# tum-pbs/differentiable-piso

Hardware: AMD Instinct MI355X
Metric: PISO steps/s (fwd+adjoint) at 2048^2 staggered grid (higher is better)
Workload: dtype f64

## Files before the change

### differentiable-piso_amd/csrc/cg.hip

```cpp
#include <atomic>
#include "cg_kernels.h"
#include "cg_driver.h"
#include "cg_tiny.h"
#include "options.h"
#include <cstdio>
#include <vector>

namespace piso {

struct CgProfile {
  int enabled = 0, stride = 8;
  double ms[4] = {0, 0, 0, 0};
  long long count[4] = {0, 0, 0, 0};
};
static CgProfile g_prof;

struct HostPoll {
  CgState* pinned = nullptr;
  hipEvent_t ev[2] = {nullptr, nullptr};
  hipEvent_t seg_ev[2] = {nullptr, nullptr};
  int cus = 0;
};
static std::atomic<unsigned> g_persist_launches{0};
static int g_persist_fallbacks = 0;
static thread_local int tl_xcd_map[kPersistMaxGrid];
static thread_local int tl_xcd_map_n = 0;
static long long g_tiny_solves = 0;
enum { DI_PATH = 0, DI_SIZEOF_T, DI_SIZEOF_CT, DI_V, DI_RECON, DI_SYMMETRIC, DI_ROWS_PER_WAVE, DI_K1_GRID, DI_K1_TILES, DI_R, DI_NQ,
       DI_WAVES, DI_LAUNCH_GRID, DI_PADDED, DI_XCD_LOCAL, DI_FELL_BACK, DI_TINY_PER_X, DI_K2_GRID, DI_SEGMENTS, DI_COUNT };
static thread_local int tl_dispatch[DI_COUNT];
static thread_local int tl_dispatch_n = 0;
static bool g_xcd_local_failed = false;
static long long g_verify_runs = 0;
static int g_verify_failures = 0;
constexpr int kPollDevices = 16;
static thread_local HostPoll tl_poll_dev[kPollDevices];
static thread_local HostPoll* tl_poll_cur = &tl_poll_dev[0];
#define tl_poll (*tl_poll_cur)

static int ensure_poll() {
  int dev = 0;
// ... 185 lines not shown
    if (prof) PISO_TRY(ensure_events(ep));
    ep.used[0] = ep.used[1] = 0;
    prof_stride = g_prof.stride > 0 ? g_prof.stride : 8;
    cg_init<T><<<tile.gflat, kBlock, 0, stream>>>(a, rank_deficient);
    PISO_LAUNCH_CHECK();
    batch = poll_batch(n);
    plan = persist_plan(PersistQuery{a.nx, a.ny, V, a.per_y, a.nx_true != 0, sizeof(T), sizeof(CT), RECON, symmetric, false, tl_poll.cus,
                                     opt(OPT_CG_PERSIST), opt(OPT_CG_PERSIST_R), opt(OPT_CG_PERSIST_HALF), opt(OPT_CG_PERSIST_NQ),
                                     opt(OPT_CG_XCD_LOCAL), g_xcd_local_failed, allow_persist});
    PISO_TRY((persist_prepare<T, CT, RECON, false>(plan, tl_poll.cus, pc, persist_ws, stream)));
    if (plan.R && kPersistDiag && opt_on(OPT_CG_PERSIST_TIMING)) {
      PISO_HIP_CHECK(hipMalloc(reinterpret_cast<void**>(&timing.ticks), 12 * plan.launch_grid * sizeof(unsigned long long)));
      PISO_HIP_CHECK(hipMemsetAsync(timing.ticks, 0, 12 * plan.launch_grid * sizeof(unsigned long long), stream));
      pc.timing = timing.ticks;
    }
    record_dispatch(plan.R ? 3 : 2, sizeof(T), sizeof(CT), 0, V, RECON, symmetric, &tile, &plan, !allow_persist);
    seg_len = persist_segment_len(n, opt(OPT_CG_SEGMENT));
    hipEvent_t* seg_ev = tl_poll.seg_ev;
    if (plan.R && prof && !seg_ev[0]) { PISO_HIP_CHECK(hipEventCreate(&seg_ev[0])); PISO_HIP_CHECK(hipEventCreate(&seg_ev[1])); }
    return PISO_OK;
  }

  bool persistent() const { return plan.R != 0; }
  int segment(int k, int ke, CgLoop& st) {
    hipEvent_t* seg_ev = tl_poll.seg_ev;
    if (prof) PISO_HIP_CHECK(hipEventRecord(seg_ev[0], stream));
    PISO_TRY((persist_launch<T, CT, RECON, false>(plan, a, pc, g_persist_launches.fetch_add(1, std::memory_order_relaxed), k, ke, st.sv, st.pending, NoSlab{}, stream)));
    if (prof) PISO_HIP_CHECK(hipEventRecord(seg_ev[1], stream));
    const bool defer = !prof && ke - k <= 32 && unsynced + (ke - k) <= 256 && ke < st.total;
    unsynced = defer ? unsynced + (ke - k) : 0;
// ... 48 lines not shown
  int look(int k, CgLoop& st) { return (!fixed && (k + 1) % batch == 0 && k + 1 < st.total) ? poll(st, false) : PISO_OK; }

  int finish(CgLoop& st) {
    if (!fixed && !st.finished) PISO_TRY(poll(st, true));
    PISO_HIP_CHECK(hipStreamSynchronize(stream));
    if (opt(OPT_CG_XCD_MAP) == 1) {
      tl_xcd_map_n = 0;
      if (st.segments_run > 0 && !plan.xcd_local && plan.grid <= kPersistMaxGrid) {
        PISO_HIP_CHECK(hipMemcpy(tl_xcd_map, pc.xcd + kPersistXcdTable, (size_t)plan.grid * sizeof(int), hipMemcpyDeviceToHost));
        tl_xcd_map_n = plan.grid;
      }
    }
    if (st.segments_run > 0) {
      int herr = 0;
      PISO_HIP_CHECK(hipMemcpy(&herr, pc.err, sizeof(int), hipMemcpyDeviceToHost));
      if (herr) { ++g_persist_fallbacks; return kPersistRetry; }
    }
    if (st.segments_run > 0 && sizeof(T) == 8 && !fixed && opt(OPT_CG_VERIFY) != 0) {
      bool failed = false;
      PISO_TRY((verify_residual<T, CT>(a, pc, stream, &failed)));
      if (failed) { ++g_verify_failures; ++g_persist_fallbacks; return kPersistRetry; }
    }
    if (timing.ticks) PISO_TRY(print_persist_timing(timing.ticks, plan.grid, st.k_last));
    tl_dispatch[DI_SEGMENTS] = st.segments_run;
    return PISO_OK;
  }
};

template <typename T>
__global__ __launch_bounds__(kBlock) void cg_copy_rows(const T* __restrict__ src, T* __restrict__ dst, int nx, int ny, int ld_src, int ld_dst) {
// ... 161 lines not shown
                                 const double* divergence, double* x_out, int rank_deficient, int iterations,
                                 float* kernel_ms_out, void* workspace, size_t workspace_bytes, piso_stream_t stream) {
  const piso::OptScope knobs;
  if (iterations < 1) { set_error_msg("piso_cg_fixed_iterations: iterations < 1"); return PISO_ERR_INVALID_ARG; }
  return cg_solve<double>(nx, ny, periodic_x, periodic_y, laplace, divergence, x_out, 0.f, iterations, rank_deficient,
                          1 << 30, iterations, nullptr, kernel_ms_out, workspace, workspace_bytes, stream);
}

void piso_cg_profile_enable(int enable, int stride) {
  g_prof.enabled = enable;
  if (stride > 0) g_prof.stride = stride;
  for (int q = 0; q < 4; ++q) { g_prof.ms[q] = 0; g_prof.count[q] = 0; }
}

int piso_cg_persist_fallbacks(void) { return g_persist_fallbacks; }
int piso_cg_last_xcd_map(int* out, int capacity) {
  const int n = tl_xcd_map_n < capacity ? tl_xcd_map_n : capacity;
  for (int i = 0; i < n; ++i) out[i] = tl_xcd_map[i];
  return tl_xcd_map_n;
}
long long piso_cg_tiny_solves(void) { return g_tiny_solves; }
int piso_cg_last_dispatch(int* out, int capacity) {
  const int n = tl_dispatch_n < capacity ? tl_dispatch_n : capacity;
  for (int i = 0; i < n; ++i) out[i] = tl_dispatch[i];
  return tl_dispatch_n;
}
void piso_cg_verify_stats(long long* runs_out, int* failures_out) {
  if (runs_out) *runs_out = g_verify_runs;
  if (failures_out) *failures_out = g_verify_failures;
}
// ... 7 lines not shown
```

### differentiable-piso_amd/csrc/cg_dispatch.h

```cpp
#pragma once
#include <type_traits>

#include "cg_persist1.h"

namespace piso {

constexpr int kXcdCus = 32;
constexpr int kPersistRetry = -1000;

struct CgTiling { int rows_per_wave, k1_tiles, g1, g2, gflat; };
template <typename T>
inline CgTiling cg_tile(CgArgs<T>& a, int V, int rpw_knob, int maxblocks_knob) {
  const size_t n = (size_t)a.nx * a.ny;
  a.ntx = (a.nx + 64 * V - 1) / (64 * V);
  int rpw = (int)(((long long)a.ny * a.ntx) / (4 * 1024));
  rpw = rpw < 2 ? 2 : (rpw > 16 ? 16 : rpw);
  if (rpw_knob > 0) rpw = rpw_knob;
  a.rows_per_wave = rpw;
  a.nty = (a.ny + 4 * rpw - 1) / (4 * rpw);
  CgTiling t;
  t.rows_per_wave = rpw; t.k1_tiles = a.ntx * a.nty;
  t.g1 = grid_for((long long)t.k1_tiles, 1, (maxblocks_knob >= 8 && maxblocks_knob <= kMaxPartials) ? maxblocks_knob : 1024);
  t.g2 = grid_for((long long)((n / V + kBlock - 1) / kBlock), 4);
  t.gflat = grid_for((long long)n, kBlock * 4);
// ... 116 lines not shown
    one(r, nq, no, no, no); one(r, nq, no, yes, no); one(r, nq, no, no, yes); one(r, nq, no, yes, yes);
    one(r, nq, yes, no, no); one(r, nq, yes, yes, no); one(r, nq, yes, no, yes); one(r, nq, yes, yes, yes);
  };
  shape(std::integral_constant<int, 2>{}, std::integral_constant<int, 1>{}); shape(std::integral_constant<int, 2>{}, std::integral_constant<int, 2>{});
  shape(std::integral_constant<int, 4>{}, std::integral_constant<int, 2>{}); shape(std::integral_constant<int, 16>{}, std::integral_constant<int, 1>{});
  return found;
}

template <typename T, typename CT, bool RECON, bool SLAB>
inline int persist_prepare(PersistPlan& p, int cus, PersistCtl& pc, unsigned* ws, hipStream_t stream) {
  int per_cu = 0;
  hipError_t e = hipSuccess;
  const bool have = persist_dispatch<T, CT, RECON, SLAB>(p, [&](auto kfn) { e = hipOccupancyMaxActiveBlocksPerMultiprocessor(&per_cu, kfn, kPersistThreads, 0); });
  if (e != hipSuccess) { set_error("hipOccupancyMaxActiveBlocksPerMultiprocessor", e); return PISO_ERR_HIP; }
  if (!have || (long long)per_cu * cus < p.launch_grid) p.R = 0;
  pc.rec = nullptr; pc.err = nullptr; pc.nreg = p.nreg; pc.ntx = p.ntx; pc.timing = nullptr; pc.epoch0 = 0; pc.xcd = nullptr; pc.local_n = 0; pc.waves = p.waves;
  if (!p.R) return PISO_OK;
  pc.rec = reinterpret_cast<unsigned long long*>(ws);
  pc.err = reinterpret_cast<int*>(ws + kPersistWsWordsAll - 16);
  pc.xcd = reinterpret_cast<int*>(ws + kPersistRecWords);
  pc.local_n = p.xcd_local ? p.grid : 0;
  PISO_HIP_CHECK(hipMemsetAsync(ws, 0, kPersistWsWordsAll * sizeof(unsigned), stream));
  return PISO_OK;
}

template <typename T, typename CT, bool RECON, bool SLAB>
inline int persist_launch(const PersistPlan& p, const CgArgs<T>& a, PersistCtl& pc, unsigned launch_count, int kb, int ke, int sv, bool pending,
                          const std::conditional_t<SLAB, SlabCtl, NoSlab>& sl, hipStream_t stream) {
  pc.epoch0 = (launch_count & 0xffffu) << 16;
  PISO_HIP_CHECK(hipMemsetAsync(pc.rec, 0, kPersistZeroBytes, stream));
  const bool have = persist_dispatch<T, CT, RECON, SLAB>(p, [&](auto kfn) { kfn<<<p.launch_grid, kPersistThreads, 0, stream>>>(a, pc, kb, ke, sv, pending ? 1 : 0, sl); });
// ... 7 lines not shown
```

### differentiable-piso_amd/csrc/cg_persist.h

```cpp
#pragma once
#include "cg_kernels.h"

#define PISO_SB_A1 __builtin_amdgcn_sched_barrier(0)
#define PISO_SB_A2 __builtin_amdgcn_sched_barrier(0)
#define PISO_SB_B1 __builtin_amdgcn_sched_barrier(0)
#define PISO_SB_B2 __builtin_amdgcn_sched_barrier(0)

namespace piso {

constexpr int kPersistThreads = 512;
constexpr int kPersistWaves = kPersistThreads / 64;

struct PersistCtl {
  unsigned long long* rec;
  int* err;
  int nreg, ntx;
  unsigned epoch0;
  unsigned long long* timing;
  int* xcd;
  int local_n;
  int waves;
};
#ifdef PISO_PERSIST_DIAG
constexpr bool kPersistDiag = true;
#else
constexpr bool kPersistDiag = false;
#endif
constexpr int kPersistMaxGrid = 256;
constexpr size_t kPersistRecWords = (size_t)2 * kPersistMaxGrid * 32 + (size_t)2 * 8 * 32;
constexpr int kPersistXcdTable = 16;
constexpr size_t kPersistWsWordsAll = kPersistRecWords + 64 + kPersistMaxGrid;
constexpr size_t kPersistZeroBytes = kPersistRecWords * 4 + 16 * sizeof(int);
constexpr int kPersistMaxDepth = 4;

__device__ __forceinline__ double read_lane_c(double v, int src) {
  const unsigned long long b = (unsigned long long)__double_as_longlong(v);
  const unsigned lo = (unsigned)__builtin_amdgcn_readlane((int)(unsigned)b, src), hi = (unsigned)__builtin_amdgcn_readlane((int)(unsigned)(b >> 32), src);
  return __longlong_as_double((long long)(((unsigned long long)hi << 32) | lo));
}
template <typename S>
__device__ __forceinline__ S uniform(S v) {
  if constexpr (sizeof(S) == 8) {
    const unsigned long long b = (unsigned long long)__double_as_longlong((double)v);
    const unsigned lo = (unsigned)__builtin_amdgcn_readfirstlane((int)(unsigned)b), hi = (unsigned)__builtin_amdgcn_readfirstlane((int)(unsigned)(b >> 32));
    return (S)__longlong_as_double((long long)(((unsigned long long)hi << 32) | lo));
// ... 95 lines not shown
```

### differentiable-piso_amd/csrc/cg_persist1.h

```cpp
#pragma once
#include <cstddef>
#include <type_traits>

#include "cg_persist.h"
#include "peer.h"

namespace piso {

struct NoSlab {};
struct SlabCtl {
  PeerView pv;
  double ncells;
  char *rows_own, *rows_lo, *rows_hi;
  unsigned hop_ticks;
};
template <typename T, typename SL>
struct Persist1Kargs { CgArgs<T> a; PersistCtl c; int k_begin, k_end, sv, pend; SL sl; };
template <typename F>
__device__ __forceinline__ F karg(unsigned off) {
  typedef __attribute__((address_space(4))) const char kchar;
  typedef __attribute__((address_space(4))) const unsigned kword;
  kchar* kp = (kchar*)__builtin_amdgcn_kernarg_segment_ptr();
  asm volatile("" : "+s"(kp));
  static_assert(sizeof(F) % 4 == 0, "whole dwords");
// ... 6 lines not shown
  __builtin_memcpy(&out, w, sizeof(F));
  return out;
}

#ifndef PISO_PERSIST1_DEPTH
#define PISO_PERSIST1_DEPTH 5
#endif
#ifndef PISO_PERSIST1_AHEAD
#define PISO_PERSIST1_AHEAD 2
#endif
#ifndef PISO_PERSIST1_KEEP_Z_REGS
#define PISO_PERSIST1_KEEP_Z_REGS 32
#endif
constexpr int kPollDelay = 24;
constexpr int kPollDelay2 = 40;
constexpr int kPollDelay2NoAhead = 8;
constexpr int kPollDelay2Xg = 8;
constexpr int kLocalDelay = 8;
constexpr int kPollSleep = 1;
constexpr int kX1Values = 8;
constexpr int kX1RecWords = 16;

constexpr int kX1Sm = 160;
struct NoPrefetch { __device__ __forceinline__ void operator()() const {} };

template <int CTRL, int BANK>
__device__ __forceinline__ double dpp_update(double old, double v) {
  const unsigned long long b = (unsigned long long)__double_as_longlong(v), o = (unsigned long long)__double_as_longlong(old);
  const unsigned lo = (unsigned)__builtin_amdgcn_update_dpp((int)(unsigned)o, (int)(unsigned)b, CTRL, 0xf, BANK, false);
  const unsigned hi = (unsigned)__builtin_amdgcn_update_dpp((int)(unsigned)(o >> 32), (int)(unsigned)(b >> 32), CTRL, 0xf, BANK, false);
// ... 154 lines not shown
  }
  __syncthreads();
  if (threadIdx.x < 64 && !lds2[1]) {
    const int xcc = lds2[0] & 7;
    int before = 0;
    for (int b = (int)threadIdx.x; b < (int)gridDim.x; b += 64)
      before += (b < (int)blockIdx.x && __hip_atomic_load(table + b, __ATOMIC_RELAXED, __HIP_MEMORY_SCOPE_AGENT) == xcc) ? 1 : 0;
#pragma unroll
    for (int off = 32; off > 0; off >>= 1) before += __shfl_xor(before, off, 64);
    if (threadIdx.x == 0) lds2[0] |= (before & 63) << 3;
  }
  __syncthreads();
  return (unsigned)__builtin_amdgcn_readfirstlane(lds2[0]);
}
constexpr int kX1SmX = 80;
template <typename T, int DELAY2, bool XG = false, typename F = NoPrefetch>
__device__ __forceinline__ bool grid_exchange8_hier(const PersistCtl& c, T (&v)[kX1Values], unsigned epoch, T* smem, unsigned hx, int* flag,
                                                    F while_records_travel = F(), unsigned long long* tsub = nullptr, unsigned sl_off = 0,
                                                    T* smx2 = nullptr) {
  unsigned long long t0 = (kPersistDiag && tsub) ? wall_clock64() : 0;
  auto tsplit = [&](int q) __attribute__((always_inline)) {
    if (kPersistDiag && tsub) { const unsigned long long t = wall_clock64(); tsub[q] += t - t0; t0 = t; }
  };
  typedef unsigned long long u64;
  constexpr int NV = kX1Values;
  const int lane = threadIdx.x & 63, wave = __builtin_amdgcn_readfirstlane(threadIdx.x >> 6);
  T* sm = smem + (epoch & 1) * kX1Sm;
  {
    double vd[NV];
#pragma unroll
    for (int q = 0; q < NV; ++q) vd[q] = (double)v[q];
    const double mine = wave_reduce_scatter8(vd);
    if (lane < NV) sm[lane * kPersistWaves + wave] = (T)mine;
  }
  asm volatile("s_waitcnt vmcnt(0)" ::: "memory");
  tsplit(0);
  __syncthreads();
  tsplit(1);
  const bool good = __builtin_amdgcn_readfirstlane(*flag) == 0;
  const unsigned spin0 = good ? 0u : (1u << 30);
  const int xcc = (int)(hx & 7u), rank = (int)((hx >> 3) & 63u), nmine = (int)((hx >> 9) & 63u);
  const unsigned present = (hx >> 15) & 0xffu;
  u64* rec1 = c.rec + (size_t)(epoch & 1) * kPersistMaxGrid * kX1RecWords + (size_t)xcc * 32 * kX1RecWords;
  u64* rec2 = hier_level2(c) + (size_t)(epoch & 1) * kXcds * kX1RecWords;
  int lw = lane;
  asm volatile("" : "+v"(lw));
  bool mygood = true;
  if (wave == 0) {
    {
      const int vq = (lane >> 1) & (NV - 1);
      T s = 0;
      for (int w = 0; w < kPersistWaves; ++w) s += sm[vq * kPersistWaves + w];
      const u64 bits = (u64)__double_as_longlong((double)s);
// ... 35 lines not shown
        const unsigned hop = karg<unsigned>(sl_off + (unsigned)offsetof(SlabCtl, hop_ticks));
        if (hop) { const unsigned long long t_go = wall_clock64() + hop; while (wall_clock64() < t_go) __builtin_amdgcn_s_sleep(1); }
        const bool lowest = (present & ((1u << xcc) - 1u)) == 0;
        for (int p = 0; p < world; ++p) {
          char* mb = karg<char*>(sl_off + pvo + (unsigned)offsetof(PeerView, mbox) + 8u * (unsigned)p);
          if (lane < kX1RecWords) peer_store(reinterpret_cast<peer_u64*>(mb + PeerLayout::xcd_rec(epoch & 1, myrank, xcc)) + lane, word);
          if (lowest && present != 0xffu) {
            for (int x = 0; x < kXcds; ++x)
              if (!((present >> x) & 1u) && lane < kX1RecWords)
                peer_store(reinterpret_cast<peer_u64*>(mb + PeerLayout::xcd_rec(epoch & 1, myrank, x)) + lane, (peer_u64)epoch);
          }
        }
      }
    }
  }
  while_records_travel();
  if constexpr (!XG) {
    u64 w[2];
    unsigned spins = spin0;
    if (DELAY2 > 0) __builtin_amdgcn_s_sleep(DELAY2);
    while (true) {
#pragma unroll
      for (int i = 0; i < 2; ++i) w[i] = __hip_atomic_load(rec2 + lw + i * 64, __ATOMIC_RELAXED, __HIP_MEMORY_SCOPE_AGENT);
      unsigned bad = 0;
#pragma unroll
      for (int i = 0; i < 2; ++i)
        bad |= (((present >> (i * 4)) >> (lw >> 4)) & 1u) ? ((unsigned)(w[i] & 0xffffffffull) ^ epoch) : 0u;
      if (__all(bad == 0)) break;
      if (++spins > (1u << 22)) { mygood = false; break; }
      __builtin_amdgcn_s_sleep(kPollSleep);
    }
    tsplit(2);
    double acc = 0;
#pragma unroll
    for (int i = 0; i < 2; ++i) {
// ... 158 lines not shown
  constexpr int ctrl = UP ? 0x138  : 0x130 ;
  if constexpr (sizeof(S) == 8) {
    const unsigned long long b = (unsigned long long)__double_as_longlong((double)v), e = (unsigned long long)__double_as_longlong((double)ring);
    const int elo = ring_to_end32<UP>((int)(unsigned)e, j), ehi = ring_to_end32<UP>((int)(unsigned)(e >> 32), j);
    const unsigned lo = (unsigned)__builtin_amdgcn_update_dpp(elo, (int)(unsigned)b, ctrl, 0xf, 0xf, false);
    const unsigned hi = (unsigned)__builtin_amdgcn_update_dpp(ehi, (int)(unsigned)(b >> 32), ctrl, 0xf, 0xf, false);
    return (S)__longlong_as_double((long long)(((unsigned long long)hi << 32) | lo));
  } else {
    const int e = ring_to_end32<UP>(__float_as_int((float)ring), j);
    return (S)__int_as_float(__builtin_amdgcn_update_dpp(e, __float_as_int((float)v), ctrl, 0xf, 0xf, false));
  }
}
__device__ __forceinline__ void ring_lane(int lane, int R, int& side, int& er) {
  side = (lane < R) ? 0 : ((lane >= 48 && lane < 48 + R) ? 1 : 2);
  er = (side == 1) ? lane - 48 : lane;
}

constexpr int kSystem = 17;

template <typename T, typename CT, int R, int NQ, bool RECON, bool SYM, bool SLAB = false, bool RAGGED = false, bool LOCAL = false>
__global__ __launch_bounds__(kPersistThreads) void cg_persist1(CgArgs<T> a, PersistCtl c, int k_begin, int k_end, int sv, int pend,
                                                               std::conditional_t<SLAB, SlabCtl, NoSlab> sl = {}) {
  static_assert(!(SLAB && RAGGED), "a slab is never padded");
  static_assert(!(SLAB && LOCAL), "a slab's neighbours are other GPUs");
  constexpr int kPub = LOCAL ? kPlain : kAgent;
  constexpr int kHalo = kAgent;
  constexpr int V = 16 / sizeof(T);
  static_assert(R * NQ <= 16 && 2 * R <= 64, "at most 16 rows per wave; the edge columns of a region fit one wave-wide load");
  static_assert(!SLAB || sizeof(T) == 8, "mailbox rows hold 8-byte elements");
  __shared__ T xs[kPersistWaves * NQ * R * 64 * V];
// ... 47 lines not shown
  if constexpr (kLocalAll) { if (threadIdx.x == 0) hier_s[2] = 0; }
  if constexpr (kHier) {
    hx = hier_enter(c, hier_s);
    if (hier_s[1]) return;
  }
  int j0[NQ], tx0[NQ];
  bool has[NQ];
#pragma unroll
  for (int q = 0; q < NQ; ++q) {
    const int reg = (wg * c.waves + wave) * NQ + q;
    has[q] = wave < c.waves && reg < c.nreg;
    const int ty = has[q] ? reg / c.ntx : 0;
    tx0[q] = has[q] ? reg - ty * c.ntx : 0;
    j0[q] = ty * R;
  }
  const unsigned nbytesT = (unsigned)((size_t)nx * ny * sizeof(T)), nbytesC = (unsigned)((size_t)nx * ny * sizeof(CT));
  const unsigned rowT = (unsigned)(nx * sizeof(T)), rowC = (unsigned)(nx * sizeof(CT));
  typedef Persist1Kargs<T, std::conditional_t<SLAB, SlabCtl, NoSlab>> KArgs;
  constexpr unsigned sl_off = (unsigned)offsetof(KArgs, sl);
  constexpr unsigned pv_off = sl_off + (unsigned)offsetof(SlabCtl, pv);
  unsigned ef[NQ];
#pragma unroll
  for (int q = 0; q < NQ; ++q) {
    ef[q] = 0;
    if constexpr (SLAB) {
      const bool bot = has[q] && j0[q] == 0, top = has[q] && j0[q] + R == ny;
      ef[q] = (bot && sl.pv.lower >= 0 ? 1u : 0u) | (top && sl.pv.upper >= 0 ? 2u : 0u) | (bot ? 4u : 0u) | (top ? 8u : 0u);
      ef[q] = (unsigned)__builtin_amdgcn_readfirstlane((int)ef[q]);
      asm volatile("" : "+s"(ef[q]));
    }
// ... 151 lines not shown
  constexpr int D = (NT >= Dw) ? Dw : NT;
  constexpr int kBaseLoads = (SYM ? 2 : 4) + (RECON ? 0 : 1);
  Vec<CT, V> cS[NT], cW[NT], cE[NT], cN[NT], cSh[NQ];
  Vec<T, V> cD[NT];
  CT eW[NQ];
  auto row_base = [&](int q, int jj, unsigned row_bytes) __attribute__((always_inline)) -> unsigned {
    unsigned j = (unsigned)j0[q];
    asm volatile("" : "+s"(j));
    return (j + (unsigned)jj) * row_bytes;
  };
  auto coef_offset = [&](int q) __attribute__((always_inline)) -> unsigned {
    return (unsigned)((unsigned long long)vT[q] * sizeof(CT) / sizeof(T));
  };
  constexpr int kAhead = (kHier && NQ == 1 && NT == 16 && SYM && RECON && sizeof(T) == 8 && sizeof(CT) == 4) ? PISO_PERSIST1_AHEAD : 0;
  static_assert(kAhead <= Dw || kAhead == 0, "the rows computed ahead are rows whose coefficients D left in registers");
  constexpr bool kShLate = kAhead > 0 && !SLAB && NQ == 1 && SYM;
  constexpr bool kKeepZ = NT * (int)sizeof(T) * V / 4 <= PISO_PERSIST1_KEEP_Z_REGS;
  constexpr bool kCountLate = NT == 16 && !RAGGED;
  auto issue_coef = [&](int t) __attribute__((always_inline)) {
    const int q = t / R, jj = t - q * R;
    const unsigned vCq = coef_offset(q);
    const unsigned sT = row_base(q, jj, rowT), sC = row_base(q, jj, rowC);
    cS[t] = bld<CT, V>(RoS, vCq, sC); cW[t] = bld<CT, V>(RoW, vCq, sC);
    if constexpr (!SYM) { cE[t] = bld<CT, V>(RoE, vCq, sC); cN[t] = bld<CT, V>(RoN, vCq, sC); }
    if constexpr (!RECON) cD[t] = bld<T, V>(RcC, vT[q], sT);
  };
  typedef __attribute__((address_space(3))) T lds_T;
  typedef __attribute__((address_space(3))) CT lds_CT;
  typedef __attribute__((address_space(3))) unsigned char lds_u8;
  unsigned ring_a = (unsigned)(unsigned long)(lds_u8*)ring_s + (unsigned)(wave * NQ * kRingBytes);
// ... 101 lines not shown
          unsigned zoff;
          const rsrc_t Rm = mailbox_rows((unsigned)offsetof(SlabCtl, rows_hi), k & 1, 0, zoff, (ef[q] & 2u) != 0);
          bst<T, V, kSystem>(Rm, vT[q], zoff, val);
        }
      }
    } else {
      if constexpr (kPack) {
        bst<T, V, kPub>(Rd, vEnd[q], row_base(q, 1, rowT) + (unsigned)(jj * 16), val);
      } else {
        bst<T, V, kPub>(Rd, vEnd[q], sT, val);
      }
    }
  };
  T eZ[NQ];
  Vec<T, V> hbZ[NQ], haZ[NQ];
  auto issue_halos = [&](rsrc_t Rz) __attribute__((always_inline)) {
#pragma unroll
    for (int q = 0; q < NQ; ++q) {
      int side, er, lane_now = lane;
      asm volatile("" : "+v"(lane_now));
      ring_lane(lane_now, R, side, er);
      int cc = (side == 0) ? tx0[q] * 64 * V - 1 : (tx0[q] + 1) * 64 * V;
      if (cc < 0) cc = a.per_x ? nx - 1 : -1;
      else if (cc >= nx) cc = a.per_x ? 0 : -1;
      unsigned vo = (side < 2 && cc >= 0) ? (unsigned)(j0[q] + er) * rowT + (unsigned)(cc * sizeof(T)) : 0xffffffffu;
      if constexpr (kPack) {
        const int strip = (cc >= 0) ? cc / (64 * V) : 0;
        const unsigned ent = (side == 0) ? (unsigned)(R * 16 + er * 16 + (V - 1) * (int)sizeof(T)) : (unsigned)(er * 16);
        vo = (side < 2 && cc >= 0) ? (unsigned)(j0[q] + 1) * rowT + (unsigned)(strip * 64 * V * (int)sizeof(T)) + ent : 0xffffffffu;
      }
      eZ[q] = bld1<T, kHalo>(Rz, vo, 0);
      bool vbq_unused, vaq_unused;
      const int jb = row_wrap(j0[q] - 1, vbq_unused), ja = row_wrap(j0[q] + R, vaq_unused);
      const bool vbq = nbit(q, 1u), vaq = nbit(q, 2u);
      if constexpr (SLAB) {
        if (!(ef[q] & 4u)) hbZ[q] = bld<T, V, kHalo>(Rz, vT[q], (unsigned)(j0[q] - 1) * rowT);
        else if (ef[q] & 1u) {
          unsigned zoff;
          const rsrc_t Rm = mailbox_rows((unsigned)offsetof(SlabCtl, rows_own), k & 1, 0, zoff);
          hbZ[q] = bld<T, V, kSystem>(Rm, vT[q], zoff);
        } else {
#pragma unroll
          for (int e = 0; e < V; ++e) hbZ[q].v[e] = 0;
        }
        if (!(ef[q] & 8u)) haZ[q] = bld<T, V, kHalo>(Rz, vT[q], (unsigned)(j0[q] + R) * rowT);
        else if (ef[q] & 2u) {
          unsigned zoff;
          const rsrc_t Rm = mailbox_rows((unsigned)offsetof(SlabCtl, rows_own), k & 1, 1, zoff);
          haZ[q] = bld<T, V, kSystem>(Rm, vT[q], zoff);
        } else {
#pragma unroll
          for (int e = 0; e < V; ++e) haZ[q].v[e] = 0;
        }
      } else {
      hbZ[q] = bld<T, V, kHalo>(make_rsrc(a.zp[k & 1], (unsigned)__builtin_amdgcn_readfirstlane((int)(vbq ? nbytesT : 0u))), vT[q], (unsigned)jb * rowT);
      haZ[q] = bld<T, V, kHalo>(make_rsrc(a.zp[k & 1], (unsigned)__builtin_amdgcn_readfirstlane((int)(vaq ? nbytesT : 0u))), vT[q], (unsigned)ja * rowT);
      }
    }
  };
  if (has[0]) {
#pragma unroll
    for (int t = 0; t < D; ++t) issue_coef(t);
  }

  unsigned epoch = c.epoch0;
  bool healthy = true, first = true;
  unsigned long long tacc[5] = {0, 0, 0, 0, 0}, tsub[4] = {0, 0, 0, 0}, tlast = (kPersistDiag && c.timing) ? wall_clock64() : 0;
  auto tick = [&](int slot) __attribute__((always_inline)) {
    if (kPersistDiag && c.timing) { const unsigned long long t = wall_clock64(); tacc[slot] += t - tlast; tlast = t; }
  };
  if (!st.done && k > 0 && (k % 5) == 0) {
// ... 72 lines not shown
    ++epoch;
    tick(0);
    Vec<T, V> zs[kAhead > 0 ? kAhead : 1];
    auto z_ahead = [&]() __attribute__((always_inline)) {
      if constexpr (kAhead > 0) {
        if (has[0]) {
          ring_issue(NT - 1);
#pragma unroll
          for (int tt = 0; tt < kAhead; ++tt) {
            if (tt + 1 < kAhead) ring_issue(NT - 2 - tt);
            zs[tt] = zrow(NT - 1 - tt);
          }
        }
      }
    };
    if constexpr (kHier) healthy = grid_exchange8_hier<T, (SLAB ? kPollDelay2Xg : (kAhead > 0 ? kPollDelay2 : kPollDelay2NoAhead)), SLAB>(c, sD, epoch, smem, hx, hier_s + 2, z_ahead, (kPersistDiag && c.timing) ? tsub : nullptr, sl_off, smem + 2 * kX1Sm);
    else if constexpr (kLocalAll) healthy = grid_exchange8_local<T>(c, sD, epoch, smem, slot, nslots, hier_s + 2, (kPersistDiag && c.timing) ? tsub : nullptr);
    else healthy = grid_exchange8<T, LOCAL>(c, sD, epoch, smem, slot, nslots, NoPrefetch(), (kPersistDiag && c.timing) ? tsub : nullptr);
    tick(1);
    if (!healthy) break;
    if (!first) {
      sumr = sD[6]; cnt_last = sD[7];
      if (k > 0 && (k % 5) == 0) {
        const int exceeded = cnt_last > 0;
        if (st.flag && !exceeded) { st.done = 1; st.iterations = k; }
        else st.flag = 1;
      }
      if (st.done) break;
    }
    first = false;
    vs = uniform(sc_c * sD[0]);
    pz = uniform(sD[2] + vs * sD[0]);
    alpha = uniform((absval(pz) > 0) ? sD[1] / pz : (T)0);
    rz_next = uniform(sD[3] - alpha * (sD[4] + vs * sD[5]));
    sumr = uniform(sumr - alpha * (sD[5] + ncells * vs));
    beta = uniform(-(rz_next + vs * sumr) / pz);
    lU[0] = 0; lU[1] = 0;
    int cnt_wave = 0;
    if (has[0]) {
      issue_halos(Rz);
      if constexpr (kAhead < NT && !kKeepZ) ring_issue(NT - 1 - kAhead);
#pragma unroll
      for (int tt = 0; tt < NT; ++tt) {
        const int t = NT - 1 - tt;
        const int q = t / R, jj = t - q * R;
        if constexpr (!kKeepZ) { if (tt + 1 < NT && tt + 1 > kAhead) ring_issue(t - 1); }
        T* xl = xs + (size_t)(wave * NQ + q) * R * 64 * V + lane * V + jj * 64 * V;
        Vec<T, V> xv = ldv<T, V>(xl);
        Vec<T, V> z;
        if constexpr (kKeepZ) z = zk[t];
        else z = (tt < kAhead) ? zs[tt < kAhead ? tt : 0] : zrow(t);
#pragma unroll
        for (int e = 0; e < V; ++e) xv.v[e] = fma(alpha, pp[q][jj].v[e], xv.v[e]);
        stv<T, V>(xl, xv);
#pragma unroll
// ... 78 lines not shown
    tOut[1] = sX[6]; tOut[2] = sX[7];
  }

  struct { T *r, *x, *pk, *partsB, *scal; const T* gB; CgState* state; int nB; } ax;
  struct { int* err; } cx;
  {
    typedef CgArgs<T> A;
    constexpr unsigned ao = (unsigned)offsetof(KArgs, a), co = (unsigned)offsetof(KArgs, c);
    ax.r = karg<T*>(ao + (unsigned)offsetof(A, r)); ax.x = karg<T*>(ao + (unsigned)offsetof(A, x));
    ax.pk = karg<T*>(ao + (unsigned)offsetof(A, p) + 8u * (unsigned)(k & 1));
    ax.partsB = karg<T*>(ao + (unsigned)offsetof(A, partsB)); ax.scal = karg<T*>(ao + (unsigned)offsetof(A, scal));
    ax.gB = karg<const T*>(ao + (unsigned)offsetof(A, gB)); ax.state = karg<CgState*>(ao + (unsigned)offsetof(A, state));
    ax.nB = karg<int>(ao + (unsigned)offsetof(A, nB));
    cx.err = karg<int*>(co + (unsigned)offsetof(PersistCtl, err));
  }
  {
    const rsrc_t Rr = make_rsrc(ax.r, nbytesT), Rx = make_rsrc(ax.x, nbytesT), Rp = make_rsrc(ax.pk, nbytesT);
#pragma unroll
    for (int q = 0; q < NQ; ++q)
      if (has[q]) {
        T* xl = xs + (size_t)(wave * NQ + q) * R * 64 * V + lane * V;
#pragma unroll
        for (int jj = 0; jj < R; ++jj) {
          const unsigned sT = (unsigned)(j0[q] + jj) * rowT;
          bst<T, V>(Rr, vT[q], sT, rr[q][jj]);
          bst<T, V>(Rp, vT[q], sT, pp[q][jj]);
          bst<T, V>(Rx, vT[q], sT, ldv<T, V>(xl + jj * 64 * V));
        }
        if constexpr (SLAB) {
          const rsrc_t RrH = make_rsrc(ax.r - nx, nbytesH), RpH = make_rsrc(ax.pk - nx, nbytesH);
// ... 25 lines not shown
```

### differentiable-piso_amd/csrc/options.h

```cpp
#pragma once

namespace piso {

enum Opt {
  OPT_CG_PERSIST = 0,
  OPT_CG_PERSIST_R,
  OPT_CG_PERSIST_HALF,
  OPT_CG_PERSIST_NQ,
  OPT_CG_SEGMENT,
  OPT_CG_PERSIST_TIMING,
  OPT_CG_RPW,
  OPT_CG_MAXBLOCKS,
  OPT_CG_NT,
  OPT_CG_NO_COMPACT,
  OPT_CG_NO_RECON,
  OPT_CG_NO_SYM,
  OPT_CG_VERIFY,
  OPT_CG_PAD,
  OPT_CG_XCD_LOCAL,
  OPT_CG_TINY,
  OPT_CG_XCD_MAP,
  OPT_CONV_LDS,
  OPT_BICG_FOLD,
  OPT_BICG_SWEEP_LDS,
  OPT_BICG_FUSE_P,
  OPT_SLAB_FORCE,
  OPT_SLAB_HOP_TICKS,
  OPT_MG_TAIL,
  OPT_MG_CHECK_EVERY,
  OPT_COUNT
};

int opt(Opt o);
inline bool opt_on(Opt o) { return opt(o) > 0; }

struct OptScope {
  OptScope();
  ~OptScope();
  OptScope(const OptScope&) = delete;
  OptScope& operator=(const OptScope&) = delete;
};

}
```

### differentiable-piso_amd/csrc/runtime.hip

```cpp
#include "piso_common.h"
#include "options.h"
#include <stdlib.h>
#include <atomic>

namespace piso {
static thread_local char g_err[512] = "";
void set_error(const char* what, hipError_t err) {
  snprintf(g_err, sizeof(g_err), "%s: %s", what, hipGetErrorString(err));
}
void set_error_msg(const char* what) { snprintf(g_err, sizeof(g_err), "%s", what); }

static const char* const kOptNames[OPT_COUNT] = {"cg_persist", "cg_persist_r", "cg_persist_half", "cg_persist_nq", "cg_segment", "cg_persist_timing",
                                                 "cg_rpw", "cg_maxblocks", "cg_nt", "cg_no_compact", "cg_no_recon", "cg_no_sym", "cg_verify", "cg_pad", "cg_xcd_local", "cg_tiny", "cg_xcd_map", "conv_lds", "bicg_fold", "bicg_sweep_lds", "bicg_fuse_p", "slab_force", "slab_hop_ticks", "mg_tail", "mg_check_every"};
struct Options {
  std::atomic<int> v[OPT_COUNT];
  Options() {
    for (int i = 0; i < OPT_COUNT; ++i) {
      char env[64] = "PISO_";
      size_t k = 5;
      for (const char* c = kOptNames[i]; *c && k + 1 < sizeof(env); ++c) env[k++] = (char)((*c >= 'a' && *c <= 'z') ? *c - 32 : *c);
      env[k] = 0;
      const char* e = getenv(env);
      v[i].store((e && *e) ? atoi(e) : -1, std::memory_order_relaxed);
    }
    if (getenv("PISO_CG_NO_PERSIST")) v[OPT_CG_PERSIST].store(0, std::memory_order_relaxed);
  }
};
static Options g_opt;
// ... 38 lines not shown
```

### differentiable-piso_amd/diffpiso/_native.py

```python
import ctypes as C
import os

import torch

_HERE = os.path.dirname(os.path.abspath(__file__))
LIB_PATH = os.environ.get("PISO_HIP_LIB") or os.path.join(_HERE, "libpiso_hip.so")

if not os.path.isfile(LIB_PATH):
    raise ImportError('HIP binaries not found at %s. Run "python differentiable-piso_amd/build_native.py" '
                      '(or __graft_entry__.build()) to compile them' % LIB_PATH)

lib = C.CDLL(LIB_PATH)

_vp, _i, _f, _sz = C.c_void_p, C.c_int, C.c_float, C.c_size_t
_ip = C.POINTER(C.c_int)

lib.piso_version.restype = C.c_char_p
lib.piso_last_error_string.restype = C.c_char_p
lib.piso_device_count.restype = _i
lib.piso_set_option.argtypes = [C.c_char_p, _i]
lib.piso_set_option.restype = _i
lib.piso_get_option.argtypes = [C.c_char_p, _ip]
lib.piso_get_option.restype = _i
lib.piso_cg_persist_fallbacks.restype = _i
lib.piso_cg_last_xcd_map.argtypes = [_ip, _i]
lib.piso_cg_last_xcd_map.restype = _i
lib.piso_cg_tiny_solves.restype = C.c_longlong
lib.piso_cg_last_dispatch.argtypes = [_ip, _i]
lib.piso_cg_last_dispatch.restype = _i
lib.piso_bicgstab_last_dispatch.argtypes = [_ip, _i]
lib.piso_bicgstab_last_dispatch.restype = _i
lib.piso_conv_last_dispatch.argtypes = [_ip, _i]
lib.piso_conv_last_dispatch.restype = _i
lib.piso_cg_verify_stats.argtypes = [C.POINTER(C.c_longlong), _ip]
lib.piso_cg_verify_stats.restype = None
lib.piso_csr_nnz.argtypes = [_i, _i, _i, _i, _ip, _ip]
lib.piso_csr_nnz.restype = None
lib.piso_assemble_csr.argtypes = [_vp, _vp, _vp, _vp, _vp, _vp, _vp, _vp, _i, _i, _i, _i, _i, _f, _f, _f, _f, _vp, _f, _vp]
lib.piso_assemble_csr.restype = _i
# ... 162 lines not shown
    return C.c_void_p(torch._C._cuda_getCurrentRawStream(torch._C._cuda_getDevice()))


_workspaces = {}


def workspace(nbytes, device, tag):
    key = (str(device), tag)
    ws = _workspaces.get(key)
    if ws is None or ws.numel() < nbytes:
        ws = torch.empty(int(nbytes), dtype=torch.uint8, device=device)
        _workspaces[key] = ws
    return ws


def cg_last_xcd_map():
    buf = (C.c_int * 256)()
    n = lib.piso_cg_last_xcd_map(buf, 256)
    return tuple(buf[i] for i in range(min(n, 256)))


def _last_dispatch(fn, name, fields):
    buf = (C.c_int * 32)()
    n = fn(buf, 32)
    if n != 0 and n != len(fields):
        raise PisoNativeError("%s returned %d fields, this binding knows %d" % (name, n, len(fields)))
    return {k: buf[i] for i, k in enumerate(fields[:n])}


DISPATCH_FIELDS = ("path", "sizeof_T", "sizeof_CT", "V", "RECON", "symmetric", "rows_per_wave", "k1_grid", "k1_tiles", "R", "NQ", "waves",
# ... 29 lines not shown
```

### include/piso_hip.h

```cpp
#ifndef PISO_HIP_H
#define PISO_HIP_H

#include <stddef.h>
#include <stdint.h>

#ifdef __cplusplus
extern "C" {
#endif

#define PISO_OK 0
#define PISO_ERR_INVALID_ARG 1
#define PISO_ERR_HIP 2
#define PISO_ERR_UNSUPPORTED_PATTERN 3
#define PISO_ERR_NO_DEVICE 4
#define PISO_ERR_NEEDS_HOST 5

typedef void* piso_stream_t;

typedef struct piso_slab {
  int ny_global;
  int row_begin, row_end;
  int owns_last_face_row;
} piso_slab_t;

// ... 88 lines not shown

int piso_cg_solve_async_f64(int nx, int ny, int periodic_x, int periodic_y, const double* laplace, const double* divergence,
                            double* x_out, float accuracy, int max_iterations, int rank_deficient, int residual_reset,
                            int* iterations_dev, void* workspace, size_t workspace_bytes, piso_stream_t stream);
int piso_cg_solve_async_f32(int nx, int ny, int periodic_x, int periodic_y, const float* laplace, const float* divergence,
                            float* x_out, float accuracy, int max_iterations, int rank_deficient, int residual_reset,
                            int* iterations_dev, void* workspace, size_t workspace_bytes, piso_stream_t stream);

int piso_cg_fixed_iterations_f64(int nx, int ny, int periodic_x, int periodic_y, const double* laplace,
                                 const double* divergence, double* x_out, int rank_deficient, int iterations,
                                 float* kernel_ms_out, void* workspace, size_t workspace_bytes, piso_stream_t stream);

void piso_cg_profile_enable(int enable, int stride);
void piso_cg_profile_read(double* ms_sum, long long* count);
int piso_cg_persist_fallbacks(void);
int piso_cg_last_xcd_map(int* out, int capacity);
long long piso_cg_tiny_solves(void);
int piso_cg_last_dispatch(int* out, int capacity);
void piso_cg_verify_stats(long long* runs_out, int* failures_out);

size_t piso_mg_workspace_bytes(int nx, int ny);
int piso_mg_pcg_solve_f64(int nx, int ny, int periodic_x, int periodic_y, const double* laplace, const double* divergence,
                          double* x_out, float accuracy, int max_iterations, int rank_deficient, int residual_reset,
                          int sweeps, int* iterations_out, void* workspace, size_t workspace_bytes, piso_stream_t stream);
int piso_mg_vcycle_f64(int nx, int ny, int periodic_x, int periodic_y, const double* laplace, const double* r_in, double* z_out,
                       int sweeps, void* workspace, size_t workspace_bytes, piso_stream_t stream);
int piso_mg_level_f64(int nx, int ny, int periodic_x, int periodic_y, const double* laplace, int level, int* nx_out, int* ny_out,
                      double* laplace_level_out, void* workspace, size_t workspace_bytes, piso_stream_t stream);
int piso_mg_last_dispatch(int* out, int capacity);

// ... 52 lines not shown
```

Before: 5.351.

## Issue CG halo loads early once neighbour records certify the epoch

In the persistent hierarchical CG kernel, each wave precomputes which exchange record certifies each neighbouring tile. While waiting on the second-level grid exchange, it polls those records and issues the top, bottom and side halo loads for its own tile as soon as the neighbours have published, instead of after the whole grid exchange. The fixed second-level sleep is replaced by a wall-clock deadline measured from publication. Early/fallback counters are exported through a new stats API. The point is to hide halo load latency behind grid synchronisation, at the cost of extra polling, LDS, register pressure, and a correctness dependence on the record-ordering certificate.

Result: slower. 5.248 (-1.9%).

```diff
diff --git a/differentiable-piso_amd/csrc/cg.hip b/differentiable-piso_amd/csrc/cg.hip
--- a/differentiable-piso_amd/csrc/cg.hip
+++ b/differentiable-piso_amd/csrc/cg.hip
@@ -25,6 +25,7 @@
 static int g_persist_fallbacks = 0;
 static thread_local int tl_xcd_map[kPersistMaxGrid];
 static thread_local int tl_xcd_map_n = 0;
+static thread_local long long tl_early_halo[2] = {0, 0};
 static long long g_tiny_solves = 0;
 enum { DI_PATH = 0, DI_SIZEOF_T, DI_SIZEOF_CT, DI_V, DI_RECON, DI_SYMMETRIC, DI_ROWS_PER_WAVE, DI_K1_GRID, DI_K1_TILES, DI_R, DI_NQ,
        DI_WAVES, DI_LAUNCH_GRID, DI_PADDED, DI_XCD_LOCAL, DI_FELL_BACK, DI_TINY_PER_X, DI_K2_GRID, DI_SEGMENTS, DI_COUNT };
@@ -240,6 +241,8 @@
       PISO_HIP_CHECK(hipMemsetAsync(timing.ticks, 0, 12 * plan.launch_grid * sizeof(unsigned long long), stream));
       pc.timing = timing.ticks;
     }
+    pc.early = opt(OPT_CG_PERSIST_EARLY_HALO) < 0 ? 0 : opt(OPT_CG_PERSIST_EARLY_HALO);
+    tl_early_halo[0] = tl_early_halo[1] = 0;
     record_dispatch(plan.R ? 3 : 2, sizeof(T), sizeof(CT), 0, V, RECON, symmetric, &tile, &plan, !allow_persist);
     seg_len = persist_segment_len(n, opt(OPT_CG_SEGMENT));
     hipEvent_t* seg_ev = tl_poll.seg_ev;
@@ -318,6 +321,9 @@
     if (st.segments_run > 0) {
       int herr = 0;
       PISO_HIP_CHECK(hipMemcpy(&herr, pc.err, sizeof(int), hipMemcpyDeviceToHost));
+      unsigned long long eh[2] = {0, 0};
+      PISO_HIP_CHECK(hipMemcpy(eh, pc.err + kPersistEarlyWords, sizeof(eh), hipMemcpyDeviceToHost));
+      tl_early_halo[0] = (long long)eh[0]; tl_early_halo[1] = (long long)eh[1];
       if (herr) { ++g_persist_fallbacks; return kPersistRetry; }
     }
     if (st.segments_run > 0 && sizeof(T) == 8 && !fixed && opt(OPT_CG_VERIFY) != 0) {
@@ -509,6 +515,10 @@
 }
 
 int piso_cg_persist_fallbacks(void) { return g_persist_fallbacks; }
+void piso_cg_early_halo_stats(long long* early_out, long long* fallback_out) {
+  if (early_out) *early_out = tl_early_halo[0];
+  if (fallback_out) *fallback_out = tl_early_halo[1];
+}
 int piso_cg_last_xcd_map(int* out, int capacity) {
   const int n = tl_xcd_map_n < capacity ? tl_xcd_map_n : capacity;
   for (int i = 0; i < n; ++i) out[i] = tl_xcd_map[i];
diff --git a/differentiable-piso_amd/csrc/cg_dispatch.h b/differentiable-piso_amd/csrc/cg_dispatch.h
--- a/differentiable-piso_amd/csrc/cg_dispatch.h
+++ b/differentiable-piso_amd/csrc/cg_dispatch.h
@@ -154,7 +154,7 @@
   const bool have = persist_dispatch<T, CT, RECON, SLAB>(p, [&](auto kfn) { e = hipOccupancyMaxActiveBlocksPerMultiprocessor(&per_cu, kfn, kPersistThreads, 0); });
   if (e != hipSuccess) { set_error("hipOccupancyMaxActiveBlocksPerMultiprocessor", e); return PISO_ERR_HIP; }
   if (!have || (long long)per_cu * cus < p.launch_grid) p.R = 0;
-  pc.rec = nullptr; pc.err = nullptr; pc.nreg = p.nreg; pc.ntx = p.ntx; pc.timing = nullptr; pc.epoch0 = 0; pc.xcd = nullptr; pc.local_n = 0; pc.waves = p.waves;
+  pc.rec = nullptr; pc.err = nullptr; pc.nreg = p.nreg; pc.ntx = p.ntx; pc.timing = nullptr; pc.epoch0 = 0; pc.xcd = nullptr; pc.local_n = 0; pc.waves = p.waves; pc.early = 0;
   if (!p.R) return PISO_OK;
   pc.rec = reinterpret_cast<unsigned long long*>(ws);
   pc.err = reinterpret_cast<int*>(ws + kPersistWsWordsAll - 16);
diff --git a/differentiable-piso_amd/csrc/cg_persist.h b/differentiable-piso_amd/csrc/cg_persist.h
--- a/differentiable-piso_amd/csrc/cg_persist.h
+++ b/differentiable-piso_amd/csrc/cg_persist.h
@@ -20,6 +20,7 @@
   int* xcd;
   int local_n;
   int waves;
+  int early;
 };
 #ifdef PISO_PERSIST_DIAG
 constexpr bool kPersistDiag = true;
@@ -29,6 +30,7 @@
 constexpr int kPersistMaxGrid = 256;
 constexpr size_t kPersistRecWords = (size_t)2 * kPersistMaxGrid * 32 + (size_t)2 * 8 * 32;
 constexpr int kPersistXcdTable = 16;
+constexpr int kPersistEarlyWords = 8;
 constexpr size_t kPersistWsWordsAll = kPersistRecWords + 64 + kPersistMaxGrid;
 constexpr size_t kPersistZeroBytes = kPersistRecWords * 4 + 16 * sizeof(int);
 constexpr int kPersistMaxDepth = 4;
diff --git a/differentiable-piso_amd/csrc/cg_persist1.h b/differentiable-piso_amd/csrc/cg_persist1.h
--- a/differentiable-piso_amd/csrc/cg_persist1.h
+++ b/differentiable-piso_amd/csrc/cg_persist1.h
@@ -44,6 +44,16 @@
 #endif
 constexpr int kPollDelay = 24;
 constexpr int kPollDelay2 = 40;
+#ifndef PISO_PERSIST1_DEADLINE2
+#define PISO_PERSIST1_DEADLINE2 140
+#endif
+#ifndef PISO_PERSIST1_CERT_FIRST
+#define PISO_PERSIST1_CERT_FIRST 1
+#endif
+constexpr int kPollDeadline2 = PISO_PERSIST1_DEADLINE2;
+constexpr int kEarlyTries = 6;
+constexpr int kEarlyUntil = kPollDeadline2 - 50;
+constexpr int kEarlySleep = 2;
 constexpr int kPollDelay2NoAhead = 8;
 constexpr int kPollDelay2Xg = 8;
 constexpr int kLocalDelay = 8;
@@ -228,10 +238,11 @@
   return (unsigned)__builtin_amdgcn_readfirstlane(lds2[0]);
 }
 constexpr int kX1SmX = 80;
-template <typename T, int DELAY2, bool XG = false, typename F = NoPrefetch>
+template <typename T, int DELAY2, bool XG = false, typename F = NoPrefetch, int DEADLINE2 = 0>
 __device__ __forceinline__ bool grid_exchange8_hier(const PersistCtl& c, T (&v)[kX1Values], unsigned epoch, T* smem, unsigned hx, int* flag,
                                                     F while_records_travel = F(), unsigned long long* tsub = nullptr, unsigned sl_off = 0,
                                                     T* smx2 = nullptr) {
+  static_assert(DEADLINE2 == 0 || !XG, "the deadline belongs to the chip's own second level");
   unsigned long long t0 = (kPersistDiag && tsub) ? wall_clock64() : 0;
   auto tsplit = [&](int q) __attribute__((always_inline)) {
     if (kPersistDiag && tsub) { const unsigned long long t = wall_clock64(); tsub[q] += t - t0; t0 = t; }
@@ -251,6 +262,7 @@
   tsplit(0);
   __syncthreads();
   tsplit(1);
+  const unsigned long long t_pub = DEADLINE2 > 0 ? wall_clock64() : 0;
   const bool good = __builtin_amdgcn_readfirstlane(*flag) == 0;
   const unsigned spin0 = good ? 0u : (1u << 30);
   const int xcc = (int)(hx & 7u), rank = (int)((hx >> 3) & 63u), nmine = (int)((hx >> 9) & 63u);
@@ -316,11 +328,14 @@
       }
     }
   }
-  while_records_travel();
+  if constexpr (DEADLINE2 > 0) while_records_travel(t_pub);
+  else while_records_travel();
   if constexpr (!XG) {
     u64 w[2];
     unsigned spins = spin0;
-    if (DELAY2 > 0) __builtin_amdgcn_s_sleep(DELAY2);
+    if constexpr (DEADLINE2 > 0) {
+      while ((unsigned)(wall_clock64() - t_pub) < (unsigned)DEADLINE2) __builtin_amdgcn_s_sleep(kPollSleep);
+    } else if (DELAY2 > 0) __builtin_amdgcn_s_sleep(DELAY2);
     while (true) {
 #pragma unroll
       for (int i = 0; i < 2; ++i) w[i] = __hip_atomic_load(rec2 + lw + i * 64, __ATOMIC_RELAXED, __HIP_MEMORY_SCOPE_AGENT);
@@ -509,6 +524,15 @@
 __device__ __forceinline__ void ring_lane(int lane, int R, int& side, int& er) {
   side = (lane < R) ? 0 : ((lane >= 48 && lane < 48 + R) ? 1 : 2);
   er = (side == 1) ? lane - 48 : lane;
+}
+
+template <typename D>
+__device__ __forceinline__ void halo_fresh(D& d) {
+  static_assert(sizeof(D) == 16 || sizeof(D) == 8, "16- or 8-byte lane accesses");
+  typedef unsigned u32x4_t __attribute__((ext_vector_type(4)));
+  typedef unsigned u32x2_t __attribute__((ext_vector_type(2)));
+  if constexpr (sizeof(D) == 16) { u32x4_t t; asm volatile("" : "=v"(t)); __builtin_memcpy(&d, &t, 16); }
+  else { u32x2_t t; asm volatile("" : "=v"(t)); __builtin_memcpy(&d, &t, 8); }
 }
 
 constexpr int kSystem = 17;
@@ -586,6 +610,38 @@
     tx0[q] = has[q] ? reg - ty * c.ntx : 0;
     j0[q] = ty * R;
   }
+  constexpr bool kEarly = kHier && !SLAB && NQ == 1 && R == 16 && SYM && RECON && sizeof(T) == 8 && sizeof(CT) == 4;
+  __shared__ int cert_s[kEarly ? kPersistWaves * 8 : 1];
+  if constexpr (kEarly) {
+    const int d = lane & 3;
+    const int nty_all = ny / R;
+    int nty = j0[0] / R + (d == 0 ? -1 : (d == 1 ? 1 : 0)), ntxn = tx0[0] + (d == 2 ? -1 : (d == 3 ? 1 : 0));
+    bool there = has[0];
+    if (nty < 0) { nty = nty_all - 1; there = there && a.per_y; }
+    if (nty >= nty_all) { nty = 0; there = there && a.per_y; }
+    if (ntxn < 0) { ntxn = c.ntx - 1; there = there && a.per_x; }
+    if (ntxn >= c.ntx) { ntxn = 0; there = there && a.per_x; }
+    const int nwg = (nty * c.ntx + ntxn) / c.waves;
+    int nb = nwg;
+    if (gridDim.x % kXcds == 0) nb = (nwg % (int)(gridDim.x / kXcds)) * kXcds + nwg / (int)(gridDim.x / kXcds);
+    int code = -1;
+    if (there && nwg != wg && nb >= 0 && nb < (int)gridDim.x) {
+      const int* table = c.xcd + kPersistXcdTable;
+      const int myx = (int)(hx & 7u);
+      const int nxcc = __hip_atomic_load(table + nb, __ATOMIC_RELAXED, __HIP_MEMORY_SCOPE_AGENT);
+      if (nxcc == myx) {
+        int before = 0;
+        for (int b = 0; b < nb; ++b) before += (__hip_atomic_load(table + b, __ATOMIC_RELAXED, __HIP_MEMORY_SCOPE_AGENT) == myx) ? 1 : 0;
+        code = ((myx * 32 + before) * kX1RecWords) << 1;
+      } else {
+        code = ((2 * kPersistMaxGrid + (nxcc & 7)) * kX1RecWords) << 1 | 1;
+      }
+    }
+    int* cs = cert_s + wave * 8;
+    if (lane < 4) cs[lane] = code;
+    if (lane == 4) cs[4] = has[0] ? c.early : 0;
+    if (lane == 5 || lane == 6) cs[lane] = 0;
+  }
   const unsigned nbytesT = (unsigned)((size_t)nx * ny * sizeof(T)), nbytesC = (unsigned)((size_t)nx * ny * sizeof(CT));
   const unsigned rowT = (unsigned)(nx * sizeof(T)), rowC = (unsigned)(nx * sizeof(CT));
   typedef Persist1Kargs<T, std::conditional_t<SLAB, SlabCtl, NoSlab>> KArgs;
@@ -767,6 +823,7 @@
   };
   constexpr int kAhead = (kHier && NQ == 1 && NT == 16 && SYM && RECON && sizeof(T) == 8 && sizeof(CT) == 4) ? PISO_PERSIST1_AHEAD : 0;
   static_assert(kAhead <= Dw || kAhead == 0, "the rows computed ahead are rows whose coefficients D left in registers");
+  static_assert(kEarly == (kAhead > 0 && !SLAB), "the window that holds the certificates is the one that computes rows ahead");
   constexpr bool kShLate = kAhead > 0 && !SLAB && NQ == 1 && SYM;
   constexpr bool kKeepZ = NT * (int)sizeof(T) * V / 4 <= PISO_PERSIST1_KEEP_Z_REGS;
   constexpr bool kCountLate = NT == 16 && !RAGGED;
@@ -898,9 +955,10 @@
   };
   T eZ[NQ];
   Vec<T, V> hbZ[NQ], haZ[NQ];
-  auto issue_halos = [&](rsrc_t Rz) __attribute__((always_inline)) {
+  auto issue_halos = [&](rsrc_t Rz, int which = 7) __attribute__((always_inline)) {
 #pragma unroll
     for (int q = 0; q < NQ; ++q) {
+      if (which & 1) {
       int side, er, lane_now = lane;
       asm volatile("" : "+v"(lane_now));
       ring_lane(lane_now, R, side, er);
@@ -914,6 +972,7 @@
         vo = (side < 2 && cc >= 0) ? (unsigned)(j0[q] + 1) * rowT + (unsigned)(strip * 64 * V * (int)sizeof(T)) + ent : 0xffffffffu;
       }
       eZ[q] = bld1<T, kHalo>(Rz, vo, 0);
+      }
       bool vbq_unused, vaq_unused;
       const int jb = row_wrap(j0[q] - 1, vbq_unused), ja = row_wrap(j0[q] + R, vaq_unused);
       const bool vbq = nbit(q, 1u), vaq = nbit(q, 2u);
@@ -937,8 +996,8 @@
           for (int e = 0; e < V; ++e) haZ[q].v[e] = 0;
         }
       } else {
-      hbZ[q] = bld<T, V, kHalo>(make_rsrc(a.zp[k & 1], (unsigned)__builtin_amdgcn_readfirstlane((int)(vbq ? nbytesT : 0u))), vT[q], (unsigned)jb * rowT);
-      haZ[q] = bld<T, V, kHalo>(make_rsrc(a.zp[k & 1], (unsigned)__builtin_amdgcn_readfirstlane((int)(vaq ? nbytesT : 0u))), vT[q], (unsigned)ja * rowT);
+      if (which & 2) hbZ[q] = bld<T, V, kHalo>(make_rsrc(a.zp[k & 1], (unsigned)__builtin_amdgcn_readfirstlane((int)(vbq ? nbytesT : 0u))), vT[q], (unsigned)jb * rowT);
+      if (which & 4) haZ[q] = bld<T, V, kHalo>(make_rsrc(a.zp[k & 1], (unsigned)__builtin_amdgcn_readfirstlane((int)(vaq ? nbytesT : 0u))), vT[q], (unsigned)ja * rowT);
       }
     }
   };
@@ -1041,7 +1100,46 @@
         }
       }
     };
-    if constexpr (kHier) healthy = grid_exchange8_hier<T, (SLAB ? kPollDelay2Xg : (kAhead > 0 ? kPollDelay2 : kPollDelay2NoAhead)), SLAB>(c, sD, epoch, smem, hx, hier_s + 2, z_ahead, (kPersistDiag && c.timing) ? tsub : nullptr, sl_off, smem + 2 * kX1Sm);
+    unsigned halo_out = 0;
+    auto window = [&](unsigned long long t_pub) __attribute__((always_inline)) {
+      if constexpr (kEarly) {
+        halo_fresh(eZ[0]); halo_fresh(hbZ[0]); halo_fresh(haZ[0]);
+#if !PISO_PERSIST1_CERT_FIRST
+        z_ahead();
+#endif
+        if (has[0]) {
+          int lane_now = lane;
+          asm volatile("" : "+v"(lane_now));
+          int* cs = cert_s + wave * 8;
+          const int code = cs[lane_now & 3];
+          const int mode = __builtin_amdgcn_readfirstlane(cs[4]);
+          if (mode != 0) {
+            const unsigned long long* rp = c.rec + (code >> 1) + (size_t)(epoch & 1) * ((code & 1) ? (size_t)kXcds * kX1RecWords : (size_t)kPersistMaxGrid * kX1RecWords);
+            for (int tries = 0; tries < kEarlyTries; ++tries) {
+              unsigned seen = epoch;
+              if (code >= 0) seen = (unsigned)(__hip_atomic_load(rp, __ATOMIC_RELAXED, __HIP_MEMORY_SCOPE_AGENT) & 0xffffffffull);
+              unsigned m = (unsigned)__ballot(seen == epoch) & 15u;
+              if (mode == 2) m = 0;
+              const unsigned ready = ((m & 12u) == 12u ? 1u : 0u) | ((m & 1u) ? 2u : 0u) | ((m & 2u) ? 4u : 0u);
+              const unsigned go = ready & ~halo_out;
+              if (go & 1u) issue_halos(Rz, 1);
+              if (go & 2u) issue_halos(Rz, 2);
+              if (go & 4u) issue_halos(Rz, 4);
+              halo_out |= go;
+              if (halo_out == 7u) break;
+              if ((unsigned)(wall_clock64() - t_pub) >= (unsigned)kEarlyUntil) break;
+              __builtin_amdgcn_s_sleep(kEarlySleep);
+            }
+            if (lane_now == 0) cs[halo_out == 7u ? 5 : 6] += 1;
+          }
+        }
+#if PISO_PERSIST1_CERT_FIRST
+        z_ahead();
+#endif
+      }
+    };
+    if constexpr (kEarly) healthy = grid_exchange8_hier<T, kPollDelay2, false, decltype(window), kPollDeadline2>(c, sD, epoch, smem, hx, hier_s + 2, window, (kPersistDiag && c.timing) ? tsub : nullptr, sl_off, smem + 2 * kX1Sm);
+    else if constexpr (kHier) healthy = grid_exchange8_hier<T, (SLAB ? kPollDelay2Xg : (kAhead > 0 ? kPollDelay2 : kPollDelay2NoAhead)), SLAB>(c, sD, epoch, smem, hx, hier_s + 2, z_ahead, (kPersistDiag && c.timing) ? tsub : nullptr, sl_off, smem + 2 * kX1Sm);
     else if constexpr (kLocalAll) healthy = grid_exchange8_local<T>(c, sD, epoch, smem, slot, nslots, hier_s + 2, (kPersistDiag && c.timing) ? tsub : nullptr);
     else healthy = grid_exchange8<T, LOCAL>(c, sD, epoch, smem, slot, nslots, NoPrefetch(), (kPersistDiag && c.timing) ? tsub : nullptr);
     tick(1);
@@ -1065,7 +1163,13 @@
     lU[0] = 0; lU[1] = 0;
     int cnt_wave = 0;
     if (has[0]) {
-      issue_halos(Rz);
+      if constexpr (kEarly) {
+        if (!(halo_out & 1u)) issue_halos(Rz, 1);
+        if (!(halo_out & 2u)) issue_halos(Rz, 2);
+        if (!(halo_out & 4u)) issue_halos(Rz, 4);
+      } else {
+        issue_halos(Rz);
+      }
       if constexpr (kAhead < NT && !kKeepZ) ring_issue(NT - 1 - kAhead);
 #pragma unroll
       for (int tt = 0; tt < NT; ++tt) {
@@ -1174,6 +1278,12 @@
     ax.nB = karg<int>(ao + (unsigned)offsetof(A, nB));
     cx.err = karg<int*>(co + (unsigned)offsetof(PersistCtl, err));
   }
+  if constexpr (kEarly) {
+    if (lane < 2 && has[0]) {
+      const int n = cert_s[wave * 8 + 5 + lane];
+      if (n) __hip_atomic_fetch_add(reinterpret_cast<unsigned long long*>(cx.err + kPersistEarlyWords) + lane, (unsigned long long)n, __ATOMIC_RELAXED, __HIP_MEMORY_SCOPE_AGENT);
+    }
+  }
   {
     const rsrc_t Rr = make_rsrc(ax.r, nbytesT), Rx = make_rsrc(ax.x, nbytesT), Rp = make_rsrc(ax.pk, nbytesT);
 #pragma unroll
diff --git a/differentiable-piso_amd/csrc/options.h b/differentiable-piso_amd/csrc/options.h
--- a/differentiable-piso_amd/csrc/options.h
+++ b/differentiable-piso_amd/csrc/options.h
@@ -28,6 +28,7 @@
   OPT_SLAB_HOP_TICKS,
   OPT_MG_TAIL,
   OPT_MG_CHECK_EVERY,
+  OPT_CG_PERSIST_EARLY_HALO,
   OPT_COUNT
 };
 
diff --git a/differentiable-piso_amd/csrc/runtime.hip b/differentiable-piso_amd/csrc/runtime.hip
--- a/differentiable-piso_amd/csrc/runtime.hip
+++ b/differentiable-piso_amd/csrc/runtime.hip
@@ -11,7 +11,7 @@
 void set_error_msg(const char* what) { snprintf(g_err, sizeof(g_err), "%s", what); }
 
 static const char* const kOptNames[OPT_COUNT] = {"cg_persist", "cg_persist_r", "cg_persist_half", "cg_persist_nq", "cg_segment", "cg_persist_timing",
-                                                 "cg_rpw", "cg_maxblocks", "cg_nt", "cg_no_compact", "cg_no_recon", "cg_no_sym", "cg_verify", "cg_pad", "cg_xcd_local", "cg_tiny", "cg_xcd_map", "conv_lds", "bicg_fold", "bicg_sweep_lds", "bicg_fuse_p", "slab_force", "slab_hop_ticks", "mg_tail", "mg_check_every"};
+                                                 "cg_rpw", "cg_maxblocks", "cg_nt", "cg_no_compact", "cg_no_recon", "cg_no_sym", "cg_verify", "cg_pad", "cg_xcd_local", "cg_tiny", "cg_xcd_map", "conv_lds", "bicg_fold", "bicg_sweep_lds", "bicg_fuse_p", "slab_force", "slab_hop_ticks", "mg_tail", "mg_check_every", "cg_persist_early_halo"};
 struct Options {
   std::atomic<int> v[OPT_COUNT];
   Options() {
diff --git a/differentiable-piso_amd/diffpiso/_native.py b/differentiable-piso_amd/diffpiso/_native.py
--- a/differentiable-piso_amd/diffpiso/_native.py
+++ b/differentiable-piso_amd/diffpiso/_native.py
@@ -23,6 +23,8 @@
 lib.piso_get_option.argtypes = [C.c_char_p, _ip]
 lib.piso_get_option.restype = _i
 lib.piso_cg_persist_fallbacks.restype = _i
+lib.piso_cg_early_halo_stats.argtypes = [C.POINTER(C.c_longlong), C.POINTER(C.c_longlong)]
+lib.piso_cg_early_halo_stats.restype = None
 lib.piso_cg_last_xcd_map.argtypes = [_ip, _i]
 lib.piso_cg_last_xcd_map.restype = _i
 lib.piso_cg_tiny_solves.restype = C.c_longlong
@@ -215,6 +217,12 @@
     return ws
 
 
+def cg_early_halo_stats():
+    early, late = C.c_longlong(0), C.c_longlong(0)
+    lib.piso_cg_early_halo_stats(C.byref(early), C.byref(late))
+    return int(early.value), int(late.value)
+
+
 def cg_last_xcd_map():
     buf = (C.c_int * 256)()
     n = lib.piso_cg_last_xcd_map(buf, 256)
diff --git a/include/piso_hip.h b/include/piso_hip.h
--- a/include/piso_hip.h
+++ b/include/piso_hip.h
@@ -126,6 +126,7 @@
 void piso_cg_profile_enable(int enable, int stride);
 void piso_cg_profile_read(double* ms_sum, long long* count);
 int piso_cg_persist_fallbacks(void);
+void piso_cg_early_halo_stats(long long* early_out, long long* fallback_out);
 int piso_cg_last_xcd_map(int* out, int capacity);
 long long piso_cg_tiny_solves(void);
 int piso_cg_last_dispatch(int* out, int capacity);
```
